# rageworx/libsrcnn

Measured on AMD Instinct MI355X. Metric: megapixels/sec SRCNN Y-channel (2x upscale), higher is better.
Workload: dtype f32

## Files before the change

### libsrcnn_amd/csrc/srcnn_kernels.hip

```cpp
#include <hip/hip_runtime.h>
#include <type_traits>
#include <stdint.h>
#include <stdlib.h>
#include <algorithm>
#include "srcnn_kernels.h"
#include "srcnn_settings.hpp"

#pragma clang fp contract(off)

namespace srcnn {

__constant__ DevWeights cW;

hipError_t upload_weights(const DevWeights& w)
{
    return hipMemcpyToSymbol(HIP_SYMBOL(cW), &w, sizeof(DevWeights));
}

__device__ __forceinline__ int clampi(int v, int lo, int hi) { return v < lo ? lo : (v > hi ? hi : v); }

__global__ __launch_bounds__(256) void k_resample_cols(
    const float* __restrict__ src, int w, int src_row_base,
    float* __restrict__ dst, int dst_row0, int dst_rows,
    const int* __restrict__ first, const int* __restrict__ taps, const double* __restrict__ wt, int stride)
// ... 309 lines not shown
    int* vn2 = vf2 + 2 * TH;
    double* mid = reinterpret_cast<double*>(vn2 + 2 * TH);
    float* raw2 = reinterpret_cast<float*>(mid + TH * LW);
    const int raw_plane = a.sr * LW;

    const int tid = threadIdx.x, lane = tid & 63, wv = __builtin_amdgcn_readfirstlane(tid >> 6);
    const int x0t = blockIdx.x * 256;
    const int xl = min(x0t + 256, a.dst_w) - 1;
    const int c0 = rs_sload(a.hfirst, x0t), cn = rs_sload(a.hfirst, xl) + rs_sload(a.htaps, xl) - c0;
    const int chunks = (cn + 63) >> 6;

    const int wr_r = tid / MAXT, wr_t = tid - wr_r * MAXT;
    double wreg = 0.0;
    int freg = 0, nreg = 0;
    auto fetch = [&](int sub) {
        const int ry0 = (blockIdx.y * a.tpb + sub) * TH;
        const int rows = min(TH, a.dst_rows - ry0);
        const int y0 = a.dst_row0 + ry0, yl = y0 + rows - 1;
        const int vmin = rs_sload(a.vfirst, y0), nsrc = rs_sload(a.vfirst, yl) + rs_sload(a.vtaps, yl) - vmin;
        if (tid < TH * MAXT && wr_r < rows) {
            const int y = y0 + wr_r;
            nreg = a.vtaps[y];
            freg = a.vfirst[y] - vmin;
            wreg = a.vwt[(size_t)y * a.vstride + min(wr_t, a.vstride - 1)];
        }
        float* raw = raw2 + (sub & 1) * raw_plane;
        const float* g = a.src_plane + (size_t)vmin * a.src_w + c0 + lane;
        for (int r = wv; r < nsrc; r += 4)
            for (int ch = 0; ch < chunks; ++ch)
                if (ch * 64 + lane < cn) rs_dma_dword(g + (size_t)r * a.src_w + ch * 64, raw + r * LW + ch * 64);
    };

    fetch(0);


    const double* hp[4][MAXT];
    double w[4][MAXT];
    int nmax = 0;
#pragma unroll
    for (int j = 0; j < 4; ++j) {
        const int xc = min(x0t + 128 * (j >> 1) + 2 * lane + (j & 1), a.dst_w - 1);
        const int s0 = a.hfirst[xc] - c0, n = a.htaps[xc];
        const double* wr = a.hwt + (size_t)xc * a.hstride;
        nmax = max(nmax, n);
#pragma unroll
        for (int t = 0; t < MAXT; ++t) {
            w[j][t] = t < n ? wr[t] : 0.0;
            hp[j][t] = mid + wv * LW + (t < n ? s0 + t : ZC);
        }
    }
    if (tid < TH) mid[tid * LW + ZC] = 0.0;
    const bool short_taps = MAXT > 1 && __builtin_amdgcn_ballot_w64(nmax > MAXT - 1) == 0;

    const int xa = x0t + 2 * lane, xb = xa + 128;
    for (int sub = 0; sub < a.tpb; ++sub) {
        const int ry0 = (blockIdx.y * a.tpb + sub) * TH;
        if (ry0 >= a.dst_rows) break;
        const int rows = min(TH, a.dst_rows - ry0);
        double* vw = vw2 + (sub & 1) * TH * MAXT;
        int* vf = vf2 + (sub & 1) * TH;
        int* vn = vn2 + (sub & 1) * TH;
        const float* raw = raw2 + (sub & 1) * raw_plane;
        if (tid < TH * MAXT && wr_r < rows) {
            vw[tid] = wr_t < nreg ? wreg : 0.0;
            if (wr_t == 0) { vf[wr_r] = freg; vn[wr_r] = nreg; }
        }
        asm volatile("s_waitcnt vmcnt(0)" ::: "memory");
        __syncthreads();
        if (sub + 1 < a.tpb && ry0 + TH < a.dst_rows) fetch(sub + 1);

        const int full = cn & ~63, rem = cn - full;
        const bool tail = rem > 0 && rem <= 16;
        const int cv = tail ? full : cn;
        for (int r = wv; r < rows; r += 4) {
            const int rb = __builtin_amdgcn_readfirstlane(vf[r]), cnt = __builtin_amdgcn_readfirstlane(vn[r]);
            double* mrow = mid + r * LW;
            const double* vwr = vw + r * MAXT;
            switch (cnt) {
#define RS_V(N) case N: if constexpr (N <= MAXT) rs_vertical_row<N, 1, MAXT, LW, double>(raw, raw_plane, mrow, vwr, rb, cv, lane); break;
            RS_V(1) RS_V(2) RS_V(3) RS_V(4) RS_V(5) RS_V(6) RS_V(7) RS_V(8)
#undef RS_V
            default: break;
            }
        }
        if (tail) {
            const int r = wv + 4 * (lane >> 4), c = full + (lane & 15);
            if (r < rows && c < cn) {
                const int rb = vf[r], cnt = vn[r];
                const double* vwr = vw + r * MAXT;
                double acc = 0.0;
#pragma unroll
                for (int t = 0; t < MAXT; ++t) {
                    const bool on = t < cnt;
                    const float xv = raw[(rb + (on ? t : 0)) * LW + c];
                    acc = acc + vwr[t] * (double)(on ? xv : 0.f);
                }
                mid[r * LW + c] = (double)(float)acc;
            }
        }
        __builtin_amdgcn_fence(__ATOMIC_RELEASE, "wavefront");
        __builtin_amdgcn_wave_barrier();
        __builtin_amdgcn_fence(__ATOMIC_ACQUIRE, "wavefront");
        auto horizontal = [&](auto ntaps) {
            constexpr int NT = decltype(ntaps)::value;
#pragma unroll
            for (int k = 0; k < RPT; ++k) {
                const int r = wv + 4 * k;
                if (r >= rows) break;
                float o[4];
#pragma unroll
                for (int j = 0; j < 4; ++j) {
                    double xs[NT];
#pragma unroll
                    for (int t = 0; t < NT; ++t) xs[t] = hp[j][t][4 * k * LW];
                    double acc = 0.0;
#pragma unroll
                    for (int t = 0; t < NT; ++t) acc = acc + w[j][t] * xs[t];
                    o[j] = (float)acc;
                }
                float* dr = a.dst + (size_t)(ry0 + r) * a.dst_w;
                if (a.vec) {
                    *reinterpret_cast<float2*>(dr + xa) = make_float2(o[0], o[1]);
                    if (xb < a.dst_w) *reinterpret_cast<float2*>(dr + xb) = make_float2(o[2], o[3]);
                } else {
                    if (xa < a.dst_w) dr[xa] = o[0];
                    if (xa + 1 < a.dst_w) dr[xa + 1] = o[1];
                    if (xb < a.dst_w) dr[xb] = o[2];
                    if (xb + 1 < a.dst_w) dr[xb + 1] = o[3];
                }
            }
        };
        if (xa < a.dst_w) {
            if (short_taps) horizontal(std::integral_constant<int, (MAXT > 1 ? MAXT - 1 : 1)>{});
            else horizontal(std::integral_constant<int, MAXT>{});
        }
        __builtin_amdgcn_fence(__ATOMIC_RELEASE, "wavefront");
        __builtin_amdgcn_wave_barrier();
        __builtin_amdgcn_fence(__ATOMIC_ACQUIRE, "wavefront");
    }
}

#define PIN(v) asm volatile("" : "+v"(v))
typedef float f32x32 __attribute__((ext_vector_type(32)));
typedef float f32x16 __attribute__((ext_vector_type(16)));

constexpr int M_NW = 8;
constexpr int M_TW = 64, M_TH = 2 * M_NW;
constexpr int M_LW = M_TW + 8;
constexpr int M_W1 = 81 * 64, M_W2 = 32 * 64, M_B1 = 64, M_B2 = 32;
constexpr int M_C1 = 32 * 32;
constexpr int M_YT = (M_TH + 8) * M_LW;
constexpr int M_BPC = 2;
static_assert(M_TH == kConv12TileRows && M_BPC == kConv12BlocksPerCU, "srcnn_kernels.h carries this geometry for the band planners");
constexpr int m_ybufs(bool ld) { return ld ? 2 : 1; }
constexpr int m_lds_floats(bool ld) { return M_W1 + M_W2 + M_B1 + M_B2 + m_ybufs(ld) * M_YT + M_NW * M_C1 + 2; }

template <int RELAX, bool LD>
__global__ __launch_bounds__(64 * M_NW, 4) void k_conv12_mfma(
    const float* __restrict__ Y, int W, int H, int y_row_base, int y_rows,
    float* __restrict__ C2, size_t plane_stride, int out_row0, int out_rows, int tiles_x, int ntiles,
    unsigned long long* __restrict__ clk, unsigned* __restrict__ queue)
{
    constexpr int NW = M_NW, NT = 64 * NW, TH = M_TH, YT = M_YT;
    unsigned long long clk_c0 = 0, clk_r0 = 0;
    if (clk && blockIdx.x == 0) { clk_c0 = __builtin_amdgcn_s_memtime(); clk_r0 = __builtin_amdgcn_s_memrealtime(); }
    constexpr bool STRICT1 = !(RELAX & 1), STRICT2 = !(RELAX & 2);
    extern __shared__ __attribute__((aligned(16))) float lds[];
    float* W1s = lds;
    float* W2s = W1s + M_W1;
    float* B1s = W2s + M_W2;
    float* B2s = B1s + M_B1;
    float* Yt  = B2s + M_B2;
    float* C1s = Yt + m_ybufs(LD) * YT;

    const int tid = threadIdx.x, lane = tid & 63, wv = tid >> 6, half = lane >> 5, col = lane & 31;

    constexpr bool WDMA = LD;
    const int wave_e0w = __builtin_amdgcn_readfirstlane(tid & ~63);
    if constexpr (WDMA) {
#pragma unroll
        for (int i = 0; i < (M_W1 + NT - 1) / NT; ++i) {
            const int e = tid + i * NT;
            if (e < M_W1) rs_dma_dword(&cW.w1t[0][0] + e, W1s + i * NT + wave_e0w);
        }
#pragma unroll
        for (int i = 0; i < (M_W2 + NT - 1) / NT; ++i) {
            const int e = tid + i * NT;
            if (e < M_W2) { const int fp = e >> 6, l = e & 63; rs_dma_dword(&cW.w2[l & 31][2 * fp + (l >> 5)], W2s + i * NT + wave_e0w); }
        }
        if (tid < 64) {
            const int hf = tid >> 5, r = tid & 31;
            rs_dma_dword(&cW.b1[32 * (r >> 4) + 8 * ((r & 15) >> 2) + 4 * hf + (r & 3)], B1s);
        }
        if (tid < 32) {
            const int hf = tid >> 4, r = tid & 15;
            rs_dma_dword(&cW.b2[8 * (r >> 2) + 4 * hf + (r & 3)], B2s);
        }
    } else {
        for (int e = tid; e < M_W1; e += NT) W1s[e] = (&cW.w1t[0][0])[e];
        for (int e = tid; e < M_W2; e += NT) {
            const int fp = e >> 6, l = e & 63;
            W2s[e] = cW.w2[l & 31][2 * fp + (l >> 5)];
        }
        if (tid < 64) {
            const int hf = tid >> 5, r = tid & 31;
            B1s[tid] = cW.b1[32 * (r >> 4) + 8 * ((r & 15) >> 2) + 4 * hf + (r & 3)];
        }
        if (tid < 32) {
            const int hf = tid >> 4, r = tid & 15;
            B2s[tid] = cW.b2[8 * (r >> 2) + 4 * hf + (r & 3)];
        }
    }
    float* myC1 = C1s + wv * M_C1;
    const f32x32 zero32 = {};

    const int full = (ntiles / (int)gridDim.x) * (int)gridDim.x;
    const int nitems = full + 4 * (ntiles - full);
    constexpr bool DMA = LD;
    constexpr int NPRE = (YT + NT - 1) / NT;
    auto tile_of = [&](int item, int& s0, int& s1) {
        int tile = item; s0 = 0; s1 = 4;
        if (item >= full) { const int i = item - full; tile = full + (i >> 2); s0 = i & 3; s1 = s0 + 1; }
        return tile;
    };
    const int wave_e0 = wave_e0w;
    auto request = [&](int item, float* buf) {
        int q0, q1;
        const int tile = tile_of(item, q0, q1);
        const int tyi = tile / tiles_x, txi = tile - tyi * tiles_x;
        const int tx0 = txi * M_TW, ty0 = out_row0 + tyi * TH;
#pragma unroll
        for (int i = 0; i < NPRE; ++i) {
            const int e = tid + i * NT;
            if (e < YT) {
                const int r = e / M_LW, c = e - r * M_LW;
                const int gy = clampi(clampi(ty0 + r - 4, 0, H - 1), y_row_base, y_row_base + y_rows - 1), gx = clampi(tx0 + c - 4, 0, W - 1);
                rs_dma_dword(Y + (size_t)(gy - y_row_base) * W + gx, buf + i * NT + wave_e0);
            }
        }
    };
    int* qslot = reinterpret_cast<int*>(C1s + NW * M_C1);
    const bool dyn = DMA && queue != nullptr;
    int it = 0;
    int item = blockIdx.x;
    if constexpr (DMA) {
        if (item < nitems) request(item, Yt);
        if (dyn && tid == 0 && item < nitems) qslot[0] = (int)gridDim.x + (int)atomicAdd(queue, 1u);
    }
    for (; item < nitems; ++it) {
        int s0, s1;
        const int tile = tile_of(item, s0, s1);
        const int tyi = tile / tiles_x, txi = tile - tyi * tiles_x;
        const int tx0 = txi * M_TW, ty0 = out_row0 + tyi * TH;
        const float* Ytc = Yt;
        int next_item = item + (int)gridDim.x;
        int drawn = 0x7fffffff;
        if constexpr (DMA) {
            Ytc = Yt + (it & 1) * YT;
            asm volatile("s_waitcnt vmcnt(0)" ::: "memory");
            __syncthreads();
            if (dyn) next_item = __builtin_amdgcn_readfirstlane(qslot[it & 1]);
            if (next_item < nitems) request(next_item, Yt + ((it + 1) & 1) * YT);
            if (dyn && tid == 0 && next_item < nitems) drawn = (int)gridDim.x + (int)atomicAdd(queue, 1u);
        } else {
            __syncthreads();
            for (int e = tid; e < YT; e += NT) {
                const int r = e / M_LW, c = e - r * M_LW;
                const int gy = clampi(clampi(ty0 + r - 4, 0, H - 1), y_row_base, y_row_base + y_rows - 1), gx = clampi(tx0 + c - 4, 0, W - 1);
                Yt[e] = Y[(size_t)(gy - y_row_base) * W + gx];
            }
            __syncthreads();
        }

#pragma unroll 1
        for (int s = s0; s < s1; ++s) {
            const int sg = wv * 4 + s;
            const int trow = sg >> 1, seg = sg & 1;
            const float* yrow = Ytc + trow * M_LW + seg * 32 + col;

            f32x32 acc = zero32;
            if constexpr (!STRICT1) {
#pragma unroll
                for (int t = 0; t < 81; ++t) {
                    const float a = W1s[t * 64 + lane];
                    const float b = yrow[(t / 9) * M_LW + (t % 9)];
                    acc = __builtin_amdgcn_mfma_f32_32x32x1f32(a, b, acc, 0, 0, 0);
                }
            } else {
                float a1 = W1s[lane], b1 = yrow[0];
                float a2 = W1s[64 + lane], b2 = yrow[1];
#pragma unroll
                for (int t = 0; t < 81; ++t) {
                    f32x32 d = __builtin_amdgcn_mfma_f32_32x32x1f32(a1, b1, zero32, 0, 0, 0);
                    PIN(d);
                    a1 = a2; b1 = b2;
                    if (t + 2 < 81) {
                        a2 = W1s[(t + 2) * 64 + lane];
                        b2 = yrow[((t + 2) / 9) * M_LW + ((t + 2) % 9)];
                    }
                    if (t == 0) acc = d; else acc += d;
                    PIN(acc);
                    __builtin_amdgcn_sched_barrier(0);
                }
            }
            f32x16 acc2 = {};
#pragma unroll
            for (int blk = 0; blk < 2; ++blk) {
#pragma unroll
                for (int r = 0; r < 16; ++r) {
                    const float v = fmaxf(acc[16 * blk + r] + B1s[half * 32 + 16 * blk + r], 0.f);
                    const int f = 8 * (r >> 2) + (r & 3);
                    myC1[(f + 4 * half) * 32 + col] = v;
                }
                __builtin_amdgcn_fence(__ATOMIC_RELEASE, "wavefront");
                __builtin_amdgcn_wave_barrier();
                __builtin_amdgcn_fence(__ATOMIC_ACQUIRE, "wavefront");

                const float* w2p = W2s + blk * 16 * 64;
                float a1 = w2p[lane], b1 = myC1[lane];
                float a2 = w2p[64 + lane], b2 = myC1[64 + lane];
                if constexpr (!STRICT2) {
#pragma unroll
                    for (int fp = 0; fp < 16; ++fp)
                        acc2 = __builtin_amdgcn_mfma_f32_32x32x2f32(w2p[fp * 64 + lane], myC1[fp * 64 + lane], acc2, 0, 0, 0);
                } else {
#pragma unroll
                    for (int fp = 0; fp < 16; ++fp) {
                        f32x32 d = __builtin_amdgcn_mfma_f32_32x32x1f32(a1, b1, zero32, 0, 0, 0);
                        PIN(d);
                        a1 = a2; b1 = b2;
                        if (fp + 2 < 16) { a2 = w2p[(fp + 2) * 64 + lane]; b2 = myC1[(fp + 2) * 64 + lane]; }
                        if (blk == 0 && fp == 0) acc2 = __builtin_shufflevector(d, d, 0, 1, 2, 3, 4, 5, 6, 7, 8, 9, 10, 11, 12, 13, 14, 15);
                        else
                        acc2 += __builtin_shufflevector(d, d, 0, 1, 2, 3, 4, 5, 6, 7, 8, 9, 10, 11, 12, 13, 14, 15);
                        acc2 += __builtin_shufflevector(d, d, 16, 17, 18, 19, 20, 21, 22, 23, 24, 25, 26, 27, 28, 29, 30, 31);
                        PIN(acc2);
                        __builtin_amdgcn_sched_barrier(0);
                    }
                }
                __builtin_amdgcn_wave_barrier();
            }

            const int row = ty0 + trow, x = tx0 + seg * 32 + col;
            if (row < out_row0 + out_rows && row < H && x < W) {
                float* dst = C2 + (size_t)(row - out_row0) * W + x;
#pragma unroll
                for (int r = 0; r < 16; ++r) {
                    const int m = 8 * (r >> 2) + (r & 3);
                    dst[(size_t)(m + 4 * half) * plane_stride] = fmaxf(acc2[r] + B2s[half * 16 + r], 0.f);
                }
            }
        }
        if (dyn && tid == 0) qslot[(it + 1) & 1] = drawn;
        item = next_item;
    }
    if (dyn && tid == 0) {
        if (atomicAdd(queue + 1, 1u) == gridDim.x - 1) { queue[0] = 0u; queue[1] = 0u; }
    }
    if (clk && blockIdx.x == 0) {
        __syncthreads();
        if (threadIdx.x == 0) {
            clk[0] = __builtin_amdgcn_s_memtime() - clk_c0;
            clk[1] = __builtin_amdgcn_s_memrealtime() - clk_r0;
        }
    }
}

constexpr int C3_TW = 64, C3_TH = 16;
constexpr int C3_LW = C3_TW + 4, C3_LH = C3_TH + 4;
constexpr int C3_CH = C3_LH * C3_LW;
static_assert(C3_LH % 4 == 0, "row slots");
constexpr int c3_mc(bool sdma) { return sdma ? 2 : 4; }

template <bool STRICT, bool OFF64 = false, bool X64 = false, bool SDMA = false>
__global__ __launch_bounds__(256, SDMA ? 6 : 3) void k_conv3(
    const float* __restrict__ C2, size_t plane_stride, int W, int H, int c2_row_base, int c2_rows,
    float* __restrict__ out, int out_row0, int out_rows, int weights_by_dma)
{
    constexpr int C3_MC = c3_mc(SDMA);
    constexpr int C3_BODY = C3_MC * C3_LH / 4;
    constexpr int C3_HALO = (C3_MC * C3_LH * 4 + 255) / 256;
    __shared__ float tile[2][C3_MC * C3_CH];
    __shared__ __attribute__((aligned(16))) float w3s[X64 ? C2N * 50 : C2N * 30];

    const int tx0 = blockIdx.x * C3_TW;
    const int ty0 = out_row0 + blockIdx.y * C3_TH;
    const int tid = threadIdx.x, lane = tid & 63, wv = tid >> 6;
    const int c2_last = c2_row_base + c2_rows - 1;
    if constexpr (X64) {
        double* w3d = reinterpret_cast<double*>(w3s);
        for (int e = tid; e < C2N * 25; e += 256) w3d[e] = (double)(&cW.w3[0][0])[e];
    } else if constexpr (STRICT) {
        const int wave_e0 = __builtin_amdgcn_readfirstlane(tid & ~63);
        if (SDMA || weights_by_dma) {
#pragma unroll
            for (int i = 0; i < (C2N * 30 + 255) / 256; ++i) {
                const int e = tid + i * 256;
                if (e < C2N * 30) rs_dma_dword(cW.w3p + e, w3s + i * 256 + wave_e0);
            }
        } else {
            for (int e = tid; e < C2N * 30; e += 256) w3s[e] = cW.w3p[e];
        }
    }

    const int bx = min(tx0 + lane, W - 1);
    const int hrow = tid >> 2, hq = tid & 3;
    const int hx = clampi(tx0 + (hq < 2 ? hq - 2 : 62 + hq), 0, W - 1);
    const int hlc = hq < 2 ? hq : 64 + hq;

    float body[C3_BODY], halo[C3_HALO];

    auto row_of = [&](int r) {
        int gy = clampi(ty0 + r - 2, 0, H - 1);
        gy = clampi(gy, c2_row_base, c2_last);
        return gy - c2_row_base;
    };
    using offs_t = std::conditional_t<OFF64, size_t, unsigned>;
    offs_t boff[C3_LH / 4], hoff[C3_HALO];
    int hm[C3_HALO];
#pragma unroll
    for (int j = 0; j < C3_LH / 4; ++j) boff[j] = ((offs_t)row_of(4 * j + wv) * (offs_t)W + (offs_t)bx) * 4u;
#pragma unroll
    for (int i = 0; i < C3_HALO; ++i) {
        const int rr = min(hrow + 64 * i, C3_MC * C3_LH - 1);
        hm[i] = rr / C3_LH;
        hoff[i] = ((offs_t)row_of(rr - hm[i] * C3_LH) * (offs_t)W + (offs_t)hx) * 4u;
    }
    const int wv_s = __builtin_amdgcn_readfirstlane(wv);
    float halo4[C3_MC];
    const int h4row = min(tid >> 2, C3_LH - 1);
    const unsigned h4off = ((unsigned)row_of(h4row) * (unsigned)W + (unsigned)hx) * 4u;
    auto issue_dma = [&](int mc, float* dst) {
        if (tid < C3_LH * 4) {
#pragma unroll
            for (int m = 0; m < C3_MC; ++m)
                halo4[m] = *reinterpret_cast<const float*>(reinterpret_cast<const char*>(C2 + (size_t)(mc + m) * plane_stride) + h4off);
        }
#pragma unroll
        for (int m = 0; m < C3_MC; ++m) {
            const unsigned long long pb = reinterpret_cast<unsigned long long>(C2 + (size_t)(mc + m) * plane_stride);
            const unsigned ub_hi = (unsigned)__builtin_amdgcn_readfirstlane((int)(unsigned)(pb >> 32));
            const unsigned ub_lo = (unsigned)__builtin_amdgcn_readfirstlane((int)(unsigned)pb);
            const unsigned long long ub = ((unsigned long long)ub_hi << 32) | (unsigned long long)ub_lo;
#pragma unroll
            for (int j = 0; j < C3_LH / 4; ++j) {
                const int i = m * (C3_LH / 4) + j;
                if constexpr (!OFF64)
                    rs_dma_dword_s(reinterpret_cast<const void*>(ub), boff[j], dst + (wv_s + 4 * i) * C3_LW + 2);
            }
        }
    };
    auto land_dma = [&](float* dst) {
        if (tid < C3_LH * 4) {
#pragma unroll
            for (int m = 0; m < C3_MC; ++m) dst[m * C3_CH + h4row * C3_LW + hlc] = halo4[m];
        }
        asm volatile("s_waitcnt vmcnt(0)" ::: "memory");
    };
    auto issue = [&](int mc) {
#pragma unroll
        for (int i = 0; i < C3_BODY; ++i) {
            const int m = i / (C3_LH / 4), j = i % (C3_LH / 4);
            const char* plane = reinterpret_cast<const char*>(C2 + (size_t)(mc + m) * plane_stride);
            body[i] = *reinterpret_cast<const float*>(plane + boff[j]);
        }
#pragma unroll
        for (int i = 0; i < C3_HALO; ++i) {
            const int rr = hrow + 64 * i;
            if (rr < C3_MC * C3_LH)
                halo[i] = *reinterpret_cast<const float*>(reinterpret_cast<const char*>(C2 + ((size_t)mc + hm[i]) * plane_stride) + hoff[i]);
        }
    };
    auto land = [&](float* dst) {
#pragma unroll
        for (int i = 0; i < C3_BODY; ++i) dst[(wv + 4 * i) * C3_LW + 2 + lane] = body[i];
#pragma unroll
        for (int i = 0; i < C3_HALO; ++i) {
            const int rr = hrow + 64 * i;
            if (rr < C3_MC * C3_LH) dst[rr * C3_LW + hlc] = halo[i];
        }
    };

    float sum[4] = {0.f, 0.f, 0.f, 0.f};

    if constexpr (SDMA) { issue_dma(0, tile[0]); land_dma(tile[0]); }
    else { issue(0); land(tile[0]); }
    if constexpr (STRICT) asm volatile("s_waitcnt vmcnt(0)" ::: "memory");
    __syncthreads();

    const int offA = (wv * 4) * C3_LW + lane;
    int offB = offA + 4 * C3_LW;
    asm volatile("" : "+v"(offB));

#pragma unroll 1
    for (int c = 0; c < C2N / C3_MC; ++c) {
        const float* cur = tile[c & 1];
        if (c + 1 < C2N / C3_MC) {
            if constexpr (SDMA) issue_dma((c + 1) * C3_MC, tile[(c + 1) & 1]);
            else issue((c + 1) * C3_MC);
        }
#pragma unroll 1
        for (int m = 0; m < C3_MC; ++m) {
// ... 312 lines not shown
constexpr int RS_LDS_LIMIT = 96 * 1024;

struct Rs2dPlan { int lw = 0, sr = 0, maxt = 0, tpb = 1; size_t lds = 0; unsigned gx = 0, gy = 0; bool ok = false; };

Rs2dPlan rs2d_plan(int np, int dst_w, int dst_row0, int dst_rows, const DevAxisTable& tv, const DevAxisTable& th, bool sliding = false)
{
    Rs2dPlan p;
    if (dst_rows <= 0 || dst_w <= 0 || !tv.monotone || !th.monotone || !tv.h_first || !th.h_first) return p;
    const int m = std::max(tv.max_taps, th.max_taps);
    if (m > 8) return p;
    p.maxt = m <= 3 ? 3 : (m <= 5 ? 5 : 8);
    int span = 0;
    for (int x0 = 0; x0 < dst_w; x0 += 256) {
        const int xl = std::min(x0 + 256, dst_w) - 1;
        span = std::max(span, th.h_first[xl] + th.h_taps[xl] - th.h_first[x0]);
    }
    p.lw = span + 1 <= 136 ? 136 : (span + 1 <= 272 ? 272 : 0);
    for (int r = 0; r < dst_rows; r += (sliding ? 1 : RS_TH)) {
        const int y0 = dst_row0 + r, yl = dst_row0 + std::min(r + RS_TH, dst_rows) - 1;
        p.sr = std::max(p.sr, tv.h_first[yl] + tv.h_taps[yl] - tv.h_first[y0]);
    }
    p.lds = (size_t)rs_lds_bytes(np, p.maxt, p.sr, p.lw);
    const unsigned tiles_y = cdiv(dst_rows, RS_TH);
    p.gx = cdiv(dst_w, 256);
    const int tpb_env = (int)settings().rs_tpb;
    p.tpb = tpb_env > 0 ? std::min(tpb_env, RS_MAX_TPB) : (int)std::max(1u, std::min<unsigned>(RS_MAX_TPB, cdiv(p.gx * tiles_y, 1024u)));
    p.gy = cdiv(tiles_y, p.tpb);
    p.ok = p.lw > 0 && p.sr > 0 && p.lds <= (size_t)RS_LDS_LIMIT && p.gy <= 65535u;
    return p;
}

template <int KIND, int D, bool CONV, class F>
void rs2d_variants(F&& f)
{
#define RS_ONE(MT, LW_) f(reinterpret_cast<const void*>(&k_rs2d<KIND, D, MT, LW_, CONV>), MT, LW_);
    RS_ONE(3, 136) RS_ONE(5, 136) RS_ONE(8, 136) RS_ONE(3, 272) RS_ONE(5, 272) RS_ONE(8, 272)
#undef RS_ONE
}

template <int KIND, int D, bool CONV>
void rs2d_dispatch(const Rs2dPlan& p, const Rs2dArgs& a, hipStream_t s)
{
    const dim3 grid(p.gx, p.gy), block(256);
#define RS_GO(MT, LW_) hipLaunchKernelGGL((k_rs2d<KIND, D, MT, LW_, CONV>), grid, block, p.lds, s, a)
    if (p.lw == 136) { if (p.maxt == 3) RS_GO(3, 136); else if (p.maxt == 5) RS_GO(5, 136); else RS_GO(8, 136); }
    else             { if (p.maxt == 3) RS_GO(3, 272); else if (p.maxt == 5) RS_GO(5, 272); else RS_GO(8, 272); }
#undef RS_GO
}
}

hipError_t rs2d_prepare()
{
    hipError_t err = hipSuccess;
    auto raise = [&](const void* fn, int, int) {
        const hipError_t e = hipFuncSetAttribute(fn, hipFuncAttributeMaxDynamicSharedMemorySize, RS_LDS_LIMIT);
        if (e != hipSuccess && err == hipSuccess) err = e;
    };
    rs2d_variants<0, 3, false>(raise);
#define RS_ONE(MT, LW_) raise(reinterpret_cast<const void*>(&k_rs2d_dma<MT, LW_>), MT, LW_);
    RS_ONE(3, 136) RS_ONE(5, 136) RS_ONE(8, 136) RS_ONE(3, 272) RS_ONE(5, 272) RS_ONE(8, 272)
#undef RS_ONE
    rs2d_variants<1, 3, false>(raise); rs2d_variants<1, 4, false>(raise);
    rs2d_variants<2, 3, false>(raise); rs2d_variants<2, 3, true>(raise);
    rs2d_variants<2, 4, false>(raise); rs2d_variants<2, 4, true>(raise);
    return err;
}

bool rs2d_fits(int np, int src_w, int src_h, int dst_w, int dst_h, int r0, int r1, const DevAxisTable& tv, const DevAxisTable& th)
{
    if (dst_w < src_w || dst_h < src_h || r1 <= r0) return false;
    const Rs2dPlan p = rs2d_plan(np, dst_w, r0, r1 - r0, tv, th, true);
    return p.lw > 0 && p.sr > 0 && p.maxt > 0 && p.lds <= (size_t)RS_LDS_LIMIT;
}

bool launch_rs2d(const YSource& src, int src_w, int src_h, float* dst, int dst_w, int dst_h, int dst_row0, int dst_rows,
                 const DevAxisTable& tv, const DevAxisTable& th, hipStream_t s)
{
    if (dst_w < src_w || dst_h < src_h) return false;
    if (!src.plane && !(src.rgb && (src.depth == 3 || src.depth == 4))) return false;
    const Rs2dPlan p = rs2d_plan(1, dst_w, dst_row0, dst_rows, tv, th);
    if (!p.ok) return false;
    Rs2dArgs a{};
    a.src_plane = src.plane; a.src_rgb = src.rgb; a.src_w = src_w;
    a.dst = dst; a.dst_w = dst_w; a.dst_row0 = dst_row0; a.dst_rows = dst_rows;
    a.sr = p.sr; a.tpb = p.tpb;
    a.vfirst = tv.first; a.vtaps = tv.taps; a.vwt = tv.weight; a.vstride = tv.stride;
    a.hfirst = th.first; a.htaps = th.taps; a.hwt = th.weight; a.hstride = th.stride;
    a.vec = (dst_w % 4 == 0) && aligned_to(dst, 16);
    const bool dma = settings().rs_dma;
    const size_t lds_dma = p.lds + (size_t)RS_TH * p.lw * 4;
    if (src.plane && dma && lds_dma <= (size_t)64 * 1024) {
        const dim3 grid(p.gx, p.gy), block(256);
#define RS_GO(MT, LW_) hipLaunchKernelGGL((k_rs2d_dma<MT, LW_>), grid, block, lds_dma, s, a)
        if (p.lw == 136) { if (p.maxt == 3) RS_GO(3, 136); else if (p.maxt == 5) RS_GO(5, 136); else RS_GO(8, 136); }
        else             { if (p.maxt == 3) RS_GO(3, 272); else if (p.maxt == 5) RS_GO(5, 272); else RS_GO(8, 272); }
#undef RS_GO
    }
    else if (src.plane) rs2d_dispatch<0, 3, false>(p, a, s);
    else if (src.depth == 3) rs2d_dispatch<1, 3, false>(p, a, s);
    else rs2d_dispatch<1, 4, false>(p, a, s);
    return true;
}

bool launch_merge_fused(const unsigned char* rgb_src, int src_w, int src_h, int depth, const float* Yp,
                        unsigned char* rgb_out, unsigned char* conv_opt, int dst_w, int dst_h, int dst_row0, int dst_rows,
                        const DevAxisTable& tv, const DevAxisTable& th, hipStream_t s)
{
    if (dst_w < src_w || dst_h < src_h || (depth != 3 && depth != 4)) return false;
    const Rs2dPlan p = rs2d_plan(depth - 1, dst_w, dst_row0, dst_rows, tv, th);
    if (!p.ok) return false;
    Rs2dArgs a{};
    a.src_rgb = rgb_src; a.src_w = src_w;
    a.yp = Yp; a.out_rgb = rgb_out; a.out_conv = conv_opt;
    a.dst_w = dst_w; a.dst_row0 = dst_row0; a.dst_rows = dst_rows;
    a.sr = p.sr; a.tpb = p.tpb;
    a.vfirst = tv.first; a.vtaps = tv.taps; a.vwt = tv.weight; a.vstride = tv.stride;
    a.hfirst = th.first; a.htaps = th.taps; a.hwt = th.weight; a.hstride = th.stride;
    a.vec = (dst_w % 4 == 0) && aligned_to(Yp, 16) && aligned_to(rgb_out, 4) && (!conv_opt || aligned_to(conv_opt, 4));
    if (depth == 3) { if (conv_opt) rs2d_dispatch<2, 3, true>(p, a, s); else rs2d_dispatch<2, 3, false>(p, a, s); }
    else            { if (conv_opt) rs2d_dispatch<2, 4, true>(p, a, s); else rs2d_dispatch<2, 4, false>(p, a, s); }
    return true;
}

template <int RELAX, bool LD>
static hipError_t prep_one()
{
    return hipFuncSetAttribute(reinterpret_cast<const void*>(&k_conv12_mfma<RELAX, LD>),
                               hipFuncAttributeMaxDynamicSharedMemorySize, (int)(sizeof(float) * m_lds_floats(LD)));
}

hipError_t conv12_mfma_prepare()
{
    hipError_t e;
    if ((e = prep_one<0, true>()) != hipSuccess) return e;
    if ((e = prep_one<0, false>()) != hipSuccess) return e;
#ifndef SRCNN_STRICT_ONLY
    if ((e = prep_one<1, true>()) != hipSuccess) return e;
    if ((e = prep_one<2, true>()) != hipSuccess) return e;
    if ((e = prep_one<3, true>()) != hipSuccess) return e;
#endif
    return hipSuccess;
}

void conv12_grid_info(int num_cus, int* blocks, int* tile_rows)
{
    if (blocks) *blocks = M_BPC * num_cus;
    if (tile_rows) *tile_rows = M_TH;
}

void launch_conv12_mfma(const float* Y, int W, int H, int y_row_base, int y_rows, float* C2, size_t plane_stride, int out_row0,
                        int out_rows, int relax, int num_cus, hipStream_t s, unsigned long long* clk, unsigned* queue)
{
    if (out_rows <= 0) return;
    const int tiles_x = (int)cdiv(W, M_TW), tiles_y = (int)cdiv(out_rows, M_TH);
    const int ntiles = tiles_x * tiles_y;
    const int cap = M_BPC * num_cus;
    const int grid = ntiles >= cap ? cap : (settings().conv12_spread ? std::min(4 * ntiles, cap) : ntiles);
#define CONV12_GO(R, LD) hipLaunchKernelGGL((k_conv12_mfma<R, LD>), dim3(grid), dim3(64 * M_NW), sizeof(float) * m_lds_floats(LD), s, Y, W, H, \
                                           y_row_base, y_rows, C2, plane_stride, out_row0, out_rows, tiles_x, ntiles, clk, LD ? queue : nullptr)
#ifdef SRCNN_STRICT_ONLY
    (void)relax;
    if (settings().conv12_dma) CONV12_GO(0, true); else CONV12_GO(0, false);
#else
    switch (relax & 3) {
    case 0: if (settings().conv12_dma) CONV12_GO(0, true); else CONV12_GO(0, false); break;
    case 1: CONV12_GO(1, true); break;
    case 2: CONV12_GO(2, true); break;
    default: CONV12_GO(3, true); break;
    }
#endif
#undef CONV12_GO
}

void launch_conv3(const float* C2, size_t plane_stride, int W, int H, int c2_row_base, int c2_rows, float* out,
                  int out_row0, int out_rows, int relax, hipStream_t s)
{
    if (out_rows <= 0) return;
#ifndef SRCNN_STRICT_ONLY
    const bool strict = !(relax & (RELAX_L3_X64 | RELAX_L3_F32));
    const bool wide_planes = (size_t)c2_rows * (size_t)W * sizeof(float) >= ((size_t)1 << 32);
    if (relax & RELAX_L3_X64) {
        const dim3 gx(cdiv(W, 64), cdiv(out_rows, 16));
        if (wide_planes)
            hipLaunchKernelGGL((k_conv3<true, true, true>), gx, dim3(256), 0, s, C2, plane_stride, W, H, c2_row_base, c2_rows, out, out_row0, out_rows, 0);
        else
            hipLaunchKernelGGL((k_conv3<true, false, true>), gx, dim3(256), 0, s, C2, plane_stride, W, H, c2_row_base, c2_rows, out, out_row0, out_rows, 0);
        return;
    }
    if (!strict) {
        dim3 gridf(cdiv(W, CF_TW), cdiv(out_rows, CF_TH));
        hipLaunchKernelGGL(k_conv3_fast, gridf, dim3(256), 0, s, C2, plane_stride, W, H, c2_row_base, c2_rows, out,
                           out_row0, out_rows);
        return;
    }
#else
    (void)relax;
#endif
    dim3 grid(cdiv(W, 64), cdiv(out_rows, 16));
    const bool force_wide = settings().conv3_off64;
    const int wdma = settings().conv3_wdma ? 1 : 0;
    const bool wide = force_wide || (size_t)c2_rows * (size_t)W * sizeof(float) >= ((size_t)1 << 32);
    if (!wide && wdma)
        hipLaunchKernelGGL((k_conv3<true, false, false, true>), grid, dim3(256), 0, s, C2, plane_stride, W, H, c2_row_base, c2_rows,
                           out, out_row0, out_rows, 1);
    else if (!wide)
        hipLaunchKernelGGL((k_conv3<true, false>), grid, dim3(256), 0, s, C2, plane_stride, W, H, c2_row_base, c2_rows,
                           out, out_row0, out_rows, wdma);
    else
        hipLaunchKernelGGL((k_conv3<true, true>), grid, dim3(256), 0, s, C2, plane_stride, W, H, c2_row_base, c2_rows,
                           out, out_row0, out_rows, wdma);
}

void launch_conv1_planes(const float* Y, int W, int H, float* C1, hipStream_t s)
{
    dim3 grid(cdiv(W, 64), cdiv(H, 4), C1N / 8);
    hipLaunchKernelGGL(k_conv1_planes, grid, dim3(256), 0, s, Y, W, H, C1, (size_t)W * H);
}

void launch_conv2_planes(const float* C1, size_t n, float* C2v, hipStream_t s)
{
    dim3 grid((unsigned)((n + 255) / 256), C2N / 8);
    hipLaunchKernelGGL(k_conv2_planes, grid, dim3(256), 0, s, C1, n, C2v);
}

template <int D>
__global__ __launch_bounds__(256) void k_rgb_split4(const unsigned* __restrict__ rgb32, size_t n4,
                                                    float4* __restrict__ Yp, float4* __restrict__ Cb,
                                                    float4* __restrict__ Cr, float4* __restrict__ A)
{
    const size_t q = (size_t)blockIdx.x * 256 + threadIdx.x;
    if (q >= n4) return;
    unsigned wds[D];
#pragma unroll
    for (int k = 0; k < D; ++k) wds[k] = rgb32[q * D + k];
    float yv[4], cbv[4], crv[4], av[4];
#pragma unroll
    for (int i = 0; i < 4; ++i) {
        float ch[4] = {0.f, 0.f, 0.f, 0.f};
#pragma unroll
        for (int k = 0; k < D; ++k) {
            const int byte = i * D + k;
            ch[k] = (float)((wds[byte >> 2] >> (8 * (byte & 3))) & 0xffu);
        }
        const float r = ch[0], g = ch[1], b = ch[2];
        yv[i] = (0.299f * r) + (0.587f * g) + (0.114f * b);
        cbv[i] = 128.f - (0.1687f * r) - (0.3313f * g) + (0.5f * b);
        crv[i] = 128.f + (0.5f * r) - (0.4187f * g) - (0.0813f * b);
        av[i] = ch[3];
    }
    Yp[q] = make_float4(yv[0], yv[1], yv[2], yv[3]);
    Cb[q] = make_float4(cbv[0], cbv[1], cbv[2], cbv[3]);
    Cr[q] = make_float4(crv[0], crv[1], crv[2], crv[3]);
    if (D == 4) A[q] = make_float4(av[0], av[1], av[2], av[3]);
}

template <int D, bool CONV>
__global__ __launch_bounds__(256) void k_ycc_merge4(const float4* __restrict__ Yp, const float4* __restrict__ Cb,
                                                    const float4* __restrict__ Cr, const float4* __restrict__ A,
                                                    size_t n4, unsigned* __restrict__ rgb32, unsigned* __restrict__ conv32)
{
    const size_t q = (size_t)blockIdx.x * 256 + threadIdx.x;
    if (q >= n4) return;
    const float4 y4 = Yp[q], cb4 = Cb[q], cr4 = Cr[q];
    float4 a4 = make_float4(0.f, 0.f, 0.f, 0.f);
    if (D == 4) a4 = A[q];
    const float ys[4] = {y4.x, y4.y, y4.z, y4.w}, cbs[4] = {cb4.x, cb4.y, cb4.z, cb4.w};
    const float crs[4] = {cr4.x, cr4.y, cr4.z, cr4.w}, as[4] = {a4.x, a4.y, a4.z, a4.w};
    unsigned wds[D] = {};
    unsigned cw = 0;
#pragma unroll
    for (int i = 0; i < 4; ++i) {
        const float fy = ys[i], cb = cbs[i] - 128.f, cr = crs[i] - 128.f;
        unsigned char px[4];
        px[0] = to_u8_sat(fy + 45.f * cr / 32.f);
        px[1] = to_u8_sat(fy - (11.f * cb + 23.f * cr) / 32.f);
        px[2] = to_u8_sat(fy + 113.f * cb / 64.f);
        px[3] = to_u8_sat(as[i]);
#pragma unroll
        for (int k = 0; k < D; ++k) {
            const int byte = i * D + k;
            wds[byte >> 2] |= (unsigned)px[k] << (8 * (byte & 3));
        }
        cw |= (unsigned)(unsigned char)fy << (8 * i);
    }
#pragma unroll
    for (int k = 0; k < D; ++k) rgb32[q * D + k] = wds[k];
    if (CONV) conv32[q] = cw;
}

static inline bool aligned16(const void* p) { return (reinterpret_cast<uintptr_t>(p) & 15u) == 0; }

void launch_rgb_split(const unsigned char* rgb, size_t n, int d, float* Yp, float* Cb, float* Cr, float* A,
                      hipStream_t s)
{
    size_t done = 0;
    if ((d == 3 || d == 4) && n >= 1024 && aligned16(Yp) && aligned16(Cb) && aligned16(Cr) && (d == 3 || aligned16(A)) &&
        (reinterpret_cast<uintptr_t>(rgb) & 3u) == 0) {
        const size_t n4 = n / 4;
        const dim3 grid((unsigned)((n4 + 255) / 256));
        if (d == 3)
            hipLaunchKernelGGL((k_rgb_split4<3>), grid, dim3(256), 0, s, reinterpret_cast<const unsigned*>(rgb), n4,
                               reinterpret_cast<float4*>(Yp), reinterpret_cast<float4*>(Cb), reinterpret_cast<float4*>(Cr),
                               reinterpret_cast<float4*>(A));
        else
            hipLaunchKernelGGL((k_rgb_split4<4>), grid, dim3(256), 0, s, reinterpret_cast<const unsigned*>(rgb), n4,
                               reinterpret_cast<float4*>(Yp), reinterpret_cast<float4*>(Cb), reinterpret_cast<float4*>(Cr),
                               reinterpret_cast<float4*>(A));
        done = n4 * 4;
    }
    if (done < n) {
        const size_t rem = n - done;
        hipLaunchKernelGGL(k_rgb_split, dim3((unsigned)((rem + 255) / 256)), dim3(256), 0, s, rgb + done * d, rem, d,
// ... 31 lines not shown
```

### libsrcnn_amd/csrc/srcnn_settings.hpp

```cpp
#pragma once
#include <cstddef>
#include <string>

#define SRCNN_SETTINGS(X)                                                                                                          \
                                                                                                            \
    X(S, devices,          "SRCNN_DEVICES",          "",    "unset = device 0, `all`, `0,1,...`", "contexts of a process that never calls `srcnn_init*` (an id may repeat: virtual contexts on one device)") \
    X(I, max_workspace_mb, "SRCNN_MAX_WORKSPACE_MB", 4608, "MiB (API twin `srcnn_set_workspace_limit`)", "layer-2 scratch one pass may hold; larger ranges are banded, bit-identically.  The default holds a whole 7680x4320 output frame (4.25 GB); lower it where memory is short: 2048 costs -1...+2 % by box, 512 +2 %, 256 +9 % (`profiles/r06_lowmem.txt`); 16384 until round 6") \
    X(I, max_lanes,        "SRCNN_MAX_LANES",        4,     "1...64", "concurrent `ProcessSRCNN` calls per context before callers queue") \
    X(B, numa,             "SRCNN_NUMA",             1,     "0/1", "place page-locked staging on the device's NUMA node (the caller's memory policy is saved and restored)") \
    X(I, comm_timeout_ms,  "SRCNN_COMM_TIMEOUT_MS",  60000, "ms, 0 = none (API twin `srcnn_comm_set_timeout_ms`)", "deadline of every wait on a peer") \
    X(B, comm_check,       "SRCNN_COMM_CHECK",       1,     "0/1", "all-reduce a checksum of every new gather table across the ranks before the first gather that uses it") \
    X(S, rccl_lib,         "SRCNN_RCCL_LIB",         "",    "path", "load this RCCL instead of the one next to the bound `libamdhip64` (site builds; the test-suite's one-device stand-in).  A trust boundary: the named file's code runs in the process; refused under secure execution (`AT_SECURE`)") \
    X(I, async_chain,      "SRCNN_ASYNC_CHAIN",      1,     "0/1/2", "order the kernels of consecutive asynchronous `ProcessSRCNN` jobs: 0 = not at all, 1 = on the host, 2 = with device-side event waits") \
    X(B, trace,            "SRCNN_TRACE",            0,     "0/1", "one stderr line per `srcnn_process_u8` share (setup / bands / stamps)") \
    X(B, roctx,            "SRCNN_ROCTX",            0,     "0/1", "roctx ranges for `rocprofv3 --marker-trace`") \
    X(S, bands,            "SRCNN_BANDS",            "",    "`f0,f1,...`", "band fractions of a large `ProcessSRCNN` image instead of the planned cuts") \
    X(I, graph_max_cpu_pct, "SRCNN_GRAPH_MAX_CPU_PCT", 10,  "0...100, 0 = never fall back", "`srcnn_y_upscale2x_f32_stream(use_graph = 1)`: hipGraph replay is kept only while the process's CPU time per replayed frame stays below this share of the frame's wall time (plain launches cost 6-8 % of a 4K frame; replay on ROCm 7.2 costs 20 % in a fresh process and ~100 % -- a runtime thread spinning from launch to completion -- in a process with more streams); above it the stream goes on with plain launches: same kernels, same overlap") \
    X(B, prefault,         "SRCNN_PREFAULT",         1,     "0/1", "pre-fault the fresh result pages of `ProcessSRCNN` in the background") \
    X(I, prefault_threads, "SRCNN_PREFAULT_THREADS", 1,     ">= 1", "helpers of that pre-faulting") \
    X(B, thp,              "SRCNN_THP",              1,     "0/1", "huge-page hint on large result blocks") \
    X(B, spin_wait,        "SRCNN_SPIN_WAIT",        0,     "0/1", "host waits through the runtime (holds a core) instead of polling") \
    X(B, device_wait_in,   "SRCNN_DEVICE_WAIT_IN",   0,     "0/1", "bands wait for their stage-in device-side (a runtime thread stays busy)") \
                   \
    X(B, conv12_queue,     "SRCNN_CONV12_QUEUE",     1,     "0/1", "layer 1+2: tiles drawn from a global counter vs dealt with a static stride") \
    X(B, conv12_dma,       "SRCNN_CONV12_DMA",       1,     "0/1", "layer 1+2: weights and Y tiles staged by LDS-DMA one tile ahead vs load, wait, `ds_write`") \
    X(B, conv12_spread,    "SRCNN_CONV12_SPREAD",    1,     "0/1", "layer 1+2: small launches dealt in quarter tiles over up to 4x more workgroups") \
    X(B, conv3_wdma,       "SRCNN_CONV3_WDMA",       1,     "0/1", "layer 3: packed weight image staged by LDS-DMA vs a plain loop") \
    X(B, conv3_off64,      "SRCNN_CONV3_OFF64",      0,     "0/1", "layer 3: 64-bit plane offsets (chosen automatically for planes of 4 GiB or more)") \
    X(B, rs_dma,           "SRCNN_RS_DMA",           1,     "0/1", "resampler: `k_rs2d_dma` (source patch by LDS-DMA) vs `k_rs2d` for plane sources") \
    X(I, rs_tpb,           "SRCNN_RS_TPB",           0,     "0 = auto, 1...16", "resampler: row tiles a block marches through") \
    X(B, resample_2pass,   "SRCNN_RESAMPLE_2PASS",   0,     "0/1", "resampler: always the two generic passes (`k_resample_cols/rows`, what down-scales use); implies the unfused colour shell") \
    X(B, shell_unfused,    "SRCNN_SHELL_UNFUSED",    0,     "0/1", "colour shell as split + plane resamples + merge instead of fused into the resampler")

namespace srcnn {

struct Settings {
#define SRCNN_SET_B(m, d) bool m = (d) != 0;
#define SRCNN_SET_I(m, d) long m = (d);
#define SRCNN_SET_S(m, d) std::string m = d;
#define X(kind, member, env, def, values, effect) SRCNN_SET_##kind(member, def)
    SRCNN_SETTINGS(X)
#undef X
#undef SRCNN_SET_B
#undef SRCNN_SET_I
#undef SRCNN_SET_S
    static Settings from_env();
    std::string describe(bool markdown) const;
};

const Settings& settings();

}
```

Before: 3571.

## Skip near-dead layer-1 channels in strict layer-2 MFMA when all zero

Adds a ballot over 15 layer-1 channels that a hardcoded mask marks as almost always zero after ReLU. When every such value in a 32-pixel segment is zero, the strict layer-2 path runs a compile-time pruned MFMA sequence over only the live channels, so it issues fewer 32x32x1 MFMAs and LDS reads. The mask is tied to the shipped weights, and the ballots plus the extra branch add work in segments where the check fails. Results should stay the same because only exact zeros are skipped, though the order of additions changes.

```diff
diff --git a/libsrcnn_amd/csrc/srcnn_kernels.hip b/libsrcnn_amd/csrc/srcnn_kernels.hip
--- a/libsrcnn_amd/csrc/srcnn_kernels.hip
+++ b/libsrcnn_amd/csrc/srcnn_kernels.hip
@@ -485,6 +485,31 @@
 constexpr int M_YT = (M_TH + 8) * M_LW;
 constexpr int M_BPC = 2;
 static_assert(M_TH == kConv12TileRows && M_BPC == kConv12BlocksPerCU, "srcnn_kernels.h carries this geometry for the band planners");
+constexpr unsigned long long M_DEAD = 0x00044e0857e40000ull;
+constexpr unsigned long long m_dead_lanes(int blk, int r)
+{
+    const int f = 32 * blk + 8 * (r >> 2) + (r & 3);
+    return ((M_DEAD >> f) & 1 ? 0x00000000ffffffffull : 0ull) | ((M_DEAD >> (f + 4)) & 1 ? 0xffffffff00000000ull : 0ull);
+}
+constexpr int m_live_count(int blk)
+{
+    int n = 0;
+    for (int f = 0; f < 32; ++f) n += !((M_DEAD >> (32 * blk + f)) & 1);
+    return n;
+}
+constexpr int m_live_nth(int blk, int n)
+{
+    for (int f = 0; f < 32; ++f)
+        if (!((M_DEAD >> (32 * blk + f)) & 1) && n-- == 0) return f;
+    return -1;
+}
+static_assert(m_live_nth(0, 0) == 0 && m_live_nth(0, 1) == 1, "the pruned body starts, like the full one, with the pair (0, 1)");
+static_assert(m_live_count(0) >= 4 && m_live_count(1) >= 4, "two pairs per block are fetched ahead");
+template <int N, class F>
+__device__ __forceinline__ void m_static_for(F&& f)
+{
+    if constexpr (N > 0) { m_static_for<N - 1>(f); f(std::integral_constant<int, N - 1>{}); }
+}
 constexpr int m_ybufs(bool ld) { return ld ? 2 : 1; }
 constexpr int m_lds_floats(bool ld) { return M_W1 + M_W2 + M_B1 + M_B2 + m_ybufs(ld) * M_YT + M_NW * M_C1 + 2; }
 
@@ -492,7 +517,7 @@
 __global__ __launch_bounds__(64 * M_NW, 4) void k_conv12_mfma(
     const float* __restrict__ Y, int W, int H, int y_row_base, int y_rows,
     float* __restrict__ C2, size_t plane_stride, int out_row0, int out_rows, int tiles_x, int ntiles,
-    unsigned long long* __restrict__ clk, unsigned* __restrict__ queue)
+    unsigned long long* __restrict__ clk, unsigned* __restrict__ queue, int prune)
 {
     constexpr int NW = M_NW, NT = 64 * NW, TH = M_TH, YT = M_YT;
     unsigned long long clk_c0 = 0, clk_r0 = 0;
@@ -639,11 +664,14 @@
             f32x16 acc2 = {};
 #pragma unroll
             for (int blk = 0; blk < 2; ++blk) {
+                unsigned long long live = 0;
 #pragma unroll
                 for (int r = 0; r < 16; ++r) {
                     const float v = fmaxf(acc[16 * blk + r] + B1s[half * 32 + 16 * blk + r], 0.f);
                     const int f = 8 * (r >> 2) + (r & 3);
                     myC1[(f + 4 * half) * 32 + col] = v;
+                    if (STRICT2 && m_dead_lanes(blk, r))
+                        live |= __builtin_amdgcn_ballot_w64((__float_as_uint(v) & 0x7fffffffu) != 0u) & m_dead_lanes(blk, r);
                 }
                 __builtin_amdgcn_fence(__ATOMIC_RELEASE, "wavefront");
                 __builtin_amdgcn_wave_barrier();
@@ -656,6 +684,32 @@
 #pragma unroll
                     for (int fp = 0; fp < 16; ++fp)
                         acc2 = __builtin_amdgcn_mfma_f32_32x32x2f32(w2p[fp * 64 + lane], myC1[fp * 64 + lane], acc2, 0, 0, 0);
+                } else if (prune && live == 0) {
+                    auto pruned = [&](auto BLK) {
+                        constexpr int B = decltype(BLK)::value, NL = m_live_count(B), NP = (NL + 1) / 2;
+                        auto off = [&](auto P) {
+                            constexpr int p = decltype(P)::value, fa = m_live_nth(B, 2 * p), fb = 2 * p + 1 < NL ? m_live_nth(B, 2 * p + 1) : fa;
+                            return lane + 32 * fa + (lane & 32) * (fb - fa - 1);
+                        };
+                        const int o0 = off(std::integral_constant<int, 0>{}), o1 = off(std::integral_constant<int, 1>{});
+                        a1 = w2p[o0]; b1 = myC1[o0];
+                        a2 = w2p[o1]; b2 = myC1[o1];
+                        m_static_for<NP>([&](auto P) {
+                            constexpr int p = decltype(P)::value;
+                            f32x32 d = __builtin_amdgcn_mfma_f32_32x32x1f32(a1, b1, zero32, 0, 0, 0);
+                            PIN(d);
+                            a1 = a2; b1 = b2;
+                            if constexpr (p + 2 < NP) { const int o = off(std::integral_constant<int, p + 2>{}); a2 = w2p[o]; b2 = myC1[o]; }
+                            if constexpr (B == 0 && p == 0) acc2 = __builtin_shufflevector(d, d, 0, 1, 2, 3, 4, 5, 6, 7, 8, 9, 10, 11, 12, 13, 14, 15);
+                            else
+                            acc2 += __builtin_shufflevector(d, d, 0, 1, 2, 3, 4, 5, 6, 7, 8, 9, 10, 11, 12, 13, 14, 15);
+                            if constexpr (2 * p + 1 < NL)
+                            acc2 += __builtin_shufflevector(d, d, 16, 17, 18, 19, 20, 21, 22, 23, 24, 25, 26, 27, 28, 29, 30, 31);
+                            PIN(acc2);
+                            __builtin_amdgcn_sched_barrier(0);
+                        });
+                    };
+                    if (blk == 0) pruned(std::integral_constant<int, 0>{}); else pruned(std::integral_constant<int, 1>{});
                 } else {
 #pragma unroll
                     for (int fp = 0; fp < 16; ++fp) {
@@ -676,11 +730,11 @@
 
             const int row = ty0 + trow, x = tx0 + seg * 32 + col;
             if (row < out_row0 + out_rows && row < H && x < W) {
-                float* dst = C2 + (size_t)(row - out_row0) * W + x;
+                float* dst = C2 + (size_t)(row - out_row0) * W + x + (size_t)(4 * half) * plane_stride;
 #pragma unroll
                 for (int r = 0; r < 16; ++r) {
                     const int m = 8 * (r >> 2) + (r & 3);
-                    dst[(size_t)(m + 4 * half) * plane_stride] = fmaxf(acc2[r] + B2s[half * 16 + r], 0.f);
+                    dst[(size_t)m * plane_stride] = fmaxf(acc2[r] + B2s[half * 16 + r], 0.f);
                 }
             }
         }
@@ -1299,12 +1353,13 @@
                         int out_rows, int relax, int num_cus, hipStream_t s, unsigned long long* clk, unsigned* queue)
 {
     if (out_rows <= 0) return;
+    const int prune = settings().conv12_prune ? 1 : 0;
     const int tiles_x = (int)cdiv(W, M_TW), tiles_y = (int)cdiv(out_rows, M_TH);
     const int ntiles = tiles_x * tiles_y;
     const int cap = M_BPC * num_cus;
     const int grid = ntiles >= cap ? cap : (settings().conv12_spread ? std::min(4 * ntiles, cap) : ntiles);
 #define CONV12_GO(R, LD) hipLaunchKernelGGL((k_conv12_mfma<R, LD>), dim3(grid), dim3(64 * M_NW), sizeof(float) * m_lds_floats(LD), s, Y, W, H, \
-                                           y_row_base, y_rows, C2, plane_stride, out_row0, out_rows, tiles_x, ntiles, clk, LD ? queue : nullptr)
+                                           y_row_base, y_rows, C2, plane_stride, out_row0, out_rows, tiles_x, ntiles, clk, LD ? queue : nullptr, prune)
 #ifdef SRCNN_STRICT_ONLY
     (void)relax;
     if (settings().conv12_dma) CONV12_GO(0, true); else CONV12_GO(0, false);
diff --git a/libsrcnn_amd/csrc/srcnn_settings.hpp b/libsrcnn_amd/csrc/srcnn_settings.hpp
--- a/libsrcnn_amd/csrc/srcnn_settings.hpp
+++ b/libsrcnn_amd/csrc/srcnn_settings.hpp
@@ -24,6 +24,7 @@
                    \
     X(B, conv12_queue,     "SRCNN_CONV12_QUEUE",     1,     "0/1", "layer 1+2: tiles drawn from a global counter vs dealt with a static stride") \
     X(B, conv12_dma,       "SRCNN_CONV12_DMA",       1,     "0/1", "layer 1+2: weights and Y tiles staged by LDS-DMA one tile ahead vs load, wait, `ds_write`") \
+    X(B, conv12_prune,     "SRCNN_CONV12_PRUNE",     1,     "0/1", "layer 1+2: strict layer 2 skips the 15 near-dead layer-1 channels in every 32-pixel segment where they are all zero vs always multiplies all 64") \
     X(B, conv12_spread,    "SRCNN_CONV12_SPREAD",    1,     "0/1", "layer 1+2: small launches dealt in quarter tiles over up to 4x more workgroups") \
     X(B, conv3_wdma,       "SRCNN_CONV3_WDMA",       1,     "0/1", "layer 3: packed weight image staged by LDS-DMA vs a plain loop") \
     X(B, conv3_off64,      "SRCNN_CONV3_OFF64",      0,     "0/1", "layer 3: 64-bit plane offsets (chosen automatically for planes of 4 GiB or more)") \
```

Measured after the change: 3722 (median of 6 runs). 1.04x the previous value.
